# BUTSpeechFIT/TS-ASR-Whisper

Hardware: AMD Instinct MI355X
Metric: train utterances/sec (30 s clips) whisper-large-v3-turbo DiCoW (higher is better)
Workload: dtype bf16; 1 GPU; whisper-large-v3-turbo DiCoW fine-tune step, per-GPU batch 16, L=128, decoder frozen, bf16 AMP; global_batch=16, parallelism=dp1, split_streams=False, trainable_params=637306880

## Files before the change

### include/dicow_hip.h

```cpp
#ifndef DICOW_HIP_H
#define DICOW_HIP_H

#include <stdint.h>

#ifdef __cplusplus
extern "C" {
#endif

#define DICOW_OK 0
#define DICOW_ERR_INVALID (-1)
#define DICOW_ERR_LAUNCH (-2)

#define DICOW_ABI_VERSION 7

int dicow_abi_version(void);
int dicow_set_gemm_cus(int n);
int dicow_gemm_dispatch_log(char* buf, int cap);
const char* dicow_last_error(void);

int dicow_cast_f32_to_bf16(const float* src, void* dst, int64_t n, void* stream);
int dicow_cast_transpose_f32_to_bf16(const float* src, void* dst, int64_t ld, void* dst_t, int64_t ld_t, int R, int C,
                                     void* stream);
#define DICOW_CAST_GROUP_MAX 8
typedef struct { const float* src; void* dst; void* dst_t; int R, C; int64_t ld, ld_t; } dicow_cast_problem;
// ... 205 lines not shown
int dicow_fabric_emulate(void* buf, int64_t bytes, double gbps, int workgroups, int passes, void* stream);
int dicow_adamw_f32(float* p, const float* g, float* m, float* v, int64_t n, float lr, float beta1, float beta2,
                    float eps, float weight_decay, int step, const float* gnorm_sq, float max_norm, void* stream);
int dicow_adamw_hyper(int* counters, float* hyper, const int* is_pre, int n_runs, int preheat_only, double lr, double mult,
                      int warmup_steps, int max_steps, int cosine, double beta1, double beta2, void* stream);
int dicow_adamw_f32_dev(float* p, const float* g, float* m, float* v, int64_t n, const float* hyper, float beta1, float beta2,
                        float eps, float weight_decay, const float* gnorm_sq, float max_norm, void* stream);

#define DICOW_MT_CHUNK 2048
#define DICOW_MT_MAX_CLASSES 32
#define DICOW_MT_ALIGNED_ALL 1
#define DICOW_MT_ALIGNED_G   2
typedef struct {
    float* p; float* g; float* m; float* v;
    int64_t n;
    int32_t cls;
    int32_t flags;
} dicow_mt_tensor;
typedef struct { int64_t start; int32_t tensor; int32_t len; } dicow_mt_chunk;
typedef struct {
    float decay[DICOW_MT_MAX_CLASSES]; float step_size[DICOW_MT_MAX_CLASSES]; float bc2_sqrt[DICOW_MT_MAX_CLASSES];
    float lerp_w[DICOW_MT_MAX_CLASSES]; float beta2[DICOW_MT_MAX_CLASSES]; float one_minus_beta2[DICOW_MT_MAX_CLASSES];
    float eps[DICOW_MT_MAX_CLASSES];
    int32_t n_classes;
} dicow_mt_adamw_classes;
int dicow_multi_chunk_elems(void);
int dicow_multi_adamw_f32(const dicow_mt_tensor* tensors, const dicow_mt_chunk* chunks, int64_t n_chunks,
                          const dicow_mt_adamw_classes* cls, int cls_base, const float* clip_coef, void* stream);
int64_t dicow_multi_sumsq_ws_bytes(int64_t n_chunks);
int dicow_multi_sumsq_f32(const dicow_mt_tensor* tensors, const dicow_mt_chunk* chunks, int64_t n_chunks, void* ws, int64_t ws_bytes,
                          float* out, float max_norm, void* stream);
int dicow_multi_scale_f32(const dicow_mt_tensor* tensors, const dicow_mt_chunk* chunks, int64_t n_chunks, const float* coef, void* stream);


#ifdef DICOW_EXPERIMENTAL_ABI
#define DICOW_EPI_LNSTAT  2048
#define DICOW_EPI_LNFOLD  4096
#define DICOW_LN_SLOTS 16
int dicow_gemm_nt_lnstat_ok(const dicow_gemm_args* a);
int dicow_lnfold_prep(const float* W, const float* gamma, const float* beta, const float* bias, void* Wf, int64_t ldw, float* c, float* bf,
                      int N, int K, void* stream);
#endif

#ifdef __cplusplus
}
#endif
#endif
```

### ts-asr-whisper_amd/_lib.py

```python
import ctypes as C
import os

_HERE = os.path.dirname(os.path.abspath(__file__))
LIB_PATH = os.environ.get("DICOW_HIP_LIB") or os.path.join(_HERE, "libdicow_hip.so")
_lib = None

c_vp, c_i, c_i64, c_f, c_d = C.c_void_p, C.c_int, C.c_int64, C.c_float, C.c_double


class FddtLnFwdArgs(C.Structure):
    _fields_ = [("h_in", c_vp), ("in_bf16", c_i), ("mode", c_i), ("stno", c_vp), ("stno_bstride", c_i64),
                ("w", c_vp * 4), ("b", c_vp * 4), ("pos", c_vp), ("h_out", c_vp), ("ln_w", c_vp), ("ln_b", c_vp),
                ("y_bf16", c_vp), ("y_f32", c_vp), ("mean", c_vp), ("rstd", c_vp),
                ("rows", c_i), ("T", c_i), ("D", c_i), ("eps", c_f)]


class FddtLnBwdArgs(C.Structure):
    _fields_ = [("h_in", c_vp), ("in_bf16", c_i), ("mode", c_i), ("stno", c_vp), ("stno_bstride", c_i64),
                ("w", c_vp * 4), ("b", c_vp * 4), ("pos", c_vp), ("ln_w", c_vp), ("mean", c_vp), ("rstd", c_vp),
                ("d_y", c_vp), ("dy_f32", c_i), ("g_res", c_vp), ("g_out", c_vp), ("g_out_bf16", c_vp),
                ("dln_w", c_vp), ("dln_b", c_vp), ("dw", c_vp * 4), ("db", c_vp * 4), ("colsum_out", c_vp),
                ("dpos_rows", c_vp), ("rows", c_i), ("T", c_i), ("D", c_i), ("ws", c_vp), ("ws_bytes", c_i64)]


# ... 98 lines not shown
    "dicow_fddt_full_combine_bwd": [c_vp, c_vp, c_i64, c_i, c_vp, c_vp, c_i, c_i, c_i, c_vp],
    "dicow_gemm_nt": [C.POINTER(GemmArgs), c_vp],
    "dicow_gemm_nt_is_persistent": [C.POINTER(GemmArgs)],
    "dicow_gemm_tn": [C.POINTER(GemmTnArgs), c_vp],
    "dicow_gemm_tn_group": [C.POINTER(GemmTnGroupArgs), c_vp],
    "dicow_attn_fwd": [C.POINTER(AttnFwdArgs), c_vp],
    "dicow_attn_bwd": [C.POINTER(AttnBwdArgs), c_vp],
    "dicow_attn_bwd_fused_status": [c_vp],
    "dicow_ce_loss_fwd": [C.POINTER(CeArgs), c_vp],
    "dicow_ce_loss_bwd": [C.POINTER(CeArgs), c_vp, c_vp],
    "dicow_ctc_loss_fwd": [C.POINTER(CtcArgs), c_vp],
    "dicow_ctc_loss_bwd": [C.POINTER(CtcArgs), c_vp, c_vp],
    "dicow_embed_fwd": [c_vp, c_vp, c_vp, c_vp, c_i, c_i, c_i, c_vp],
    "dicow_embed_bwd": [c_vp, c_vp, c_vp, c_vp, c_i, c_i, c_i, c_vp],
    "dicow_gelu_bwd_bf16": [c_vp, c_vp, c_vp, c_i64, c_vp],
    "dicow_conv2_col2im_gelu_bwd": [c_vp, c_vp, c_vp, c_i, c_i, c_i, c_vp],
    "dicow_logmel": [c_vp, c_i, c_i, c_vp, c_vp, c_vp, c_vp, c_i, c_vp, c_vp, c_i64, c_vp],
    "dicow_stno_noise_rescale": [c_vp, c_vp, c_vp, c_i, c_i, c_i, c_f, c_vp],
    "dicow_stno_segment_augment": [c_vp, c_vp, c_vp, c_i, c_i, c_i, c_vp],
    "dicow_specaug_joint": [c_vp, c_vp, c_vp, c_vp, c_i, c_i, c_i, c_i, c_i, c_i, c_vp, c_i, c_vp, c_i, c_i, c_vp],
    "dicow_ctc_frame_lse": [c_vp, c_i, c_i64, c_i, c_i64, c_vp, c_vp],
    "dicow_ctc_prefix_init": [c_vp, c_i, c_i64, c_vp, c_i, c_i, c_i, c_vp, c_vp],
    "dicow_ctc_prefix_score": [C.POINTER(CtcPrefixArgs), c_vp],
    "dicow_whisper_timestamp_rules": [c_vp, c_i64, c_i, c_i, c_vp, c_i, c_i, c_i, c_i, c_i, c_i, c_i, c_vp],
    "dicow_sumsq_f32": [c_vp, c_i64, c_vp, c_vp],
    "dicow_fabric_emulate": [c_vp, c_i64, c_d, c_i, c_i, c_vp],
    "dicow_adamw_f32": [c_vp, c_vp, c_vp, c_vp, c_i64, c_f, c_f, c_f, c_f, c_f, c_i, c_vp, c_f, c_vp],
    "dicow_adamw_hyper": [c_vp, c_vp, c_vp, c_i, c_i, c_d, c_d, c_i, c_i, c_i, c_d, c_d, c_vp],
    "dicow_adamw_f32_dev": [c_vp, c_vp, c_vp, c_vp, c_i64, c_vp, c_f, c_f, c_f, c_f, c_vp, c_f, c_vp],
    "dicow_multi_chunk_elems": [],
    "dicow_multi_adamw_f32": [c_vp, c_vp, c_i64, C.POINTER(MtAdamwClasses), c_i, c_vp, c_vp],
    "dicow_multi_sumsq_f32": [c_vp, c_vp, c_i64, c_vp, c_i64, c_vp, c_f, c_vp],
    "dicow_multi_scale_f32": [c_vp, c_vp, c_i64, c_vp, c_vp],
}


_SIGS_EXPERIMENTAL = {
    "dicow_gemm_nt_lnstat_ok": [C.POINTER(GemmArgs)],
    "dicow_lnfold_prep": [c_vp, c_vp, c_vp, c_vp, c_vp, c_i64, c_vp, c_vp, c_i, c_i, c_vp],
}


class DicowError(RuntimeError):
    pass


def lib():
    global _lib
    if _lib is None:
        if not os.path.exists(LIB_PATH):
            raise DicowError(f"{LIB_PATH} is missing: build it with ts-asr-whisper_amd/csrc/build.sh "
                             "(or __graft_entry__.build()); there is no CPU fallback")
        l = C.CDLL(LIB_PATH)
        l.dicow_abi_version.restype = c_i
        l.dicow_last_error.restype = C.c_char_p
        for name, at in _SIGS.items():
            fn = getattr(l, name)
            fn.argtypes = at
            fn.restype = c_i
        for name, at in _SIGS64.items():
            fn = getattr(l, name)
            fn.argtypes = at
            fn.restype = c_i64
        for name, at in _SIGS_STR.items():
            fn = getattr(l, name)
            fn.argtypes = at
# ... 65 lines not shown
```

### ts-asr-whisper_amd/csrc/elementwise.hip

```cpp
#include <stdarg.h>
#include "common.h"

static thread_local char g_err[512] = "";

void dicow_set_error(const char* fmt, ...) {
    va_list ap;
    va_start(ap, fmt);
    vsnprintf(g_err, sizeof(g_err), fmt, ap);
    va_end(ap);
}

extern "C" int dicow_abi_version(void) { return DICOW_ABI_VERSION; }
extern "C" const char* dicow_last_error(void) { return g_err; }

__global__ void cast_f32_bf16_kernel(const float* __restrict__ src, unsigned short* __restrict__ dst, int64_t n) {
    const int64_t n4 = n >> 2;
    const int64_t stride = (int64_t)gridDim.x * blockDim.x;
    for (int64_t i = (int64_t)blockIdx.x * blockDim.x + threadIdx.x; i < n4; i += stride) {
        const float4 v = reinterpret_cast<const float4*>(src)[i];
        reinterpret_cast<uint2*>(dst)[i] = make_uint2(pack_bf16x2(v.x, v.y), pack_bf16x2(v.z, v.w));
    }
    for (int64_t i = (n4 << 2) + (int64_t)blockIdx.x * blockDim.x + threadIdx.x; i < n; i += stride)
        dst[i] = f2bfbits(src[i]);
}

extern "C" int dicow_cast_f32_to_bf16(const float* src, void* dst, int64_t n, void* stream) {
    DICOW_REQUIRE(src && dst && n > 0, "cast_f32_to_bf16: bad args");
    int grid = (int)((n / 4 + 255) / 256);
    if (grid < 1) grid = 1;
    if (grid > 4096) grid = 4096;
    hipLaunchKernelGGL(cast_f32_bf16_kernel, dim3(grid), dim3(256), 0, (hipStream_t)stream, src, (unsigned short*)dst, n);
    DICOW_CHECK_LAUNCH("cast_f32_to_bf16");
    return DICOW_OK;
// ... 216 lines not shown
        }
        reinterpret_cast<float4*>(out)[i] = s;
    }
}
struct reduce_multi_args { float* out[11]; };
__global__ void reduce_parts_tall_kernel(const float* __restrict__ part, int nparts, int64_t stride, int64_t kstride,
                                         reduce_multi_args outs, int64_t n) {
    __shared__ float red[16][17];
    float* out = outs.out[blockIdx.y];
    if (!out) return;
    part += (int64_t)blockIdx.y * kstride;
    const int c = threadIdx.x & 15, pl = threadIdx.x >> 4;
    const int64_t j = (int64_t)blockIdx.x * 16 + c;
    float s = 0.f;
    if (j < n) {
        int p = pl;
        for (; p + 48 < nparts; p += 64) {
            const float a0 = part[(int64_t)p * stride + j], a1 = part[(int64_t)(p + 16) * stride + j];
            const float a2 = part[(int64_t)(p + 32) * stride + j], a3 = part[(int64_t)(p + 48) * stride + j];
            s += (a0 + a1) + (a2 + a3);
        }
        for (; p < nparts; p += 16) s += part[(int64_t)p * stride + j];
    }
    red[pl][c] = s;
    __syncthreads();
    if (pl == 0 && j < n) {
        float t = 0.f;
#pragma unroll
        for (int q = 0; q < 16; ++q) t += red[q][c];
        out[j] += t;
    }
}

int dicow_launch_reduce_multi(const float* part, int nparts, int64_t stride, int64_t kstride, float* const* outs, int nout,
                              int64_t n, hipStream_t st) {
#ifdef DICOW_SKIP_REDUCE_MULTI
    return DICOW_OK;
#endif
    reduce_multi_args ra;
    for (int k = 0; k < 11; ++k) ra.out[k] = k < nout ? outs[k] : nullptr;
    hipLaunchKernelGGL(reduce_parts_tall_kernel, dim3((unsigned)((n + 15) / 16), nout), dim3(256), 0, st, part, nparts, stride,
                       kstride, ra, n);
    DICOW_CHECK_LAUNCH("reduce_parts_multi");
    return DICOW_OK;
}

int dicow_launch_reduce_parts(const float* part, int nparts, int64_t stride, float* out, int64_t n, hipStream_t st) {
    if (nparts <= 16 && n % 4 == 0 && stride % 4 == 0) {
        int grid = (int)((n / 4 + 255) / 256); if (grid > 4096) grid = 4096; if (grid < 1) grid = 1;
        hipLaunchKernelGGL(reduce_parts_wide_kernel, dim3(grid), dim3(256), 0, st, part, nparts, stride, out, n / 4);
    } else {
        float* outs[1] = {out};
        return dicow_launch_reduce_multi(part, nparts, stride, 0, outs, 1, n, st);
    }
    DICOW_CHECK_LAUNCH("reduce_parts");
    return DICOW_OK;
}

__global__ void colsum_bf16_kernel(const unsigned short* __restrict__ x, int64_t ld, float* __restrict__ part, int rows, int N) {
    const int c = (blockIdx.x * blockDim.x + threadIdx.x) * 2;
    if (c >= N) return;
    float s0 = 0.f, s1 = 0.f;
    const int r1 = (int)(((int64_t)rows * (blockIdx.y + 1)) / gridDim.y);
    for (int r = (int)(((int64_t)rows * blockIdx.y) / gridDim.y); r < r1; ++r) {
        const unsigned u = *reinterpret_cast<const unsigned*>(x + (int64_t)r * ld + c);
        s0 += __uint_as_float(u << 16);
        s1 += __uint_as_float(u & 0xffff0000u);
    }
    *reinterpret_cast<float2*>(part + (int64_t)blockIdx.y * N + c) = make_float2(s0, s1);
}

static int colsum_slices(int rows, int N) {
    const int gx = dicow_cdiv(N, 512);
    int gy = 2048 / gx; if (gy < 1) gy = 1; if (gy > rows) gy = rows; if (gy > 512) gy = 512;
    return gy;
}

extern "C" int64_t dicow_colsum_ws_bytes(int rows, int N) { return (int64_t)colsum_slices(rows, N) * N * 4; }

extern "C" int dicow_colsum_bf16(const void* x, int64_t ld, float* out, int rows, int N, void* ws, int64_t ws_bytes, void* stream) {
    DICOW_REQUIRE(x && out && rows > 0 && N > 0 && N % 2 == 0 && ld % 2 == 0, "colsum_bf16: bad args (N, ld must be even)");
    const int gx = dicow_cdiv(N, 512), gy = colsum_slices(rows, N);
    DICOW_REQUIRE(ws && ws_bytes >= (int64_t)gy * N * 4, "colsum_bf16: workspace too small (need %ld bytes)", (long)gy * N * 4);
    hipLaunchKernelGGL(colsum_bf16_kernel, dim3(gx, gy), dim3(256), 0, (hipStream_t)stream, (const unsigned short*)x, ld, (float*)ws, rows, N);
    DICOW_CHECK_LAUNCH("colsum_bf16");
    return dicow_launch_reduce_parts((const float*)ws, gy, N, out, N, (hipStream_t)stream);
}

__global__ void sum_over_batch_kernel(const float* __restrict__ g, float* __restrict__ out, int B, int64_t TD) {
// ... 463 lines not shown
```

### ts-asr-whisper_amd/engine.py

```python
import contextlib
import os
from types import SimpleNamespace as NS

import torch

from . import _lib as L
from . import ops

BF16, F32 = torch.bfloat16, torch.float32
CLS = ("silence_linear", "target_linear", "non_target_linear", "overlap_linear")


def _e(shape, dtype, dev):
    return torch.empty(shape, dtype=dtype, device=dev)


def _ceil(a, b):
    return (a + b - 1) // b * b


WGRAD_SIDE_STREAM = os.environ.get("DICOW_WGRAD_STREAM", "0") == "1"
WGRAD_STREAM_PRIORITY = int(os.environ.get("DICOW_WGRAD_STREAM_PRIORITY", "-1"))
_WGRAD_STREAMS = {}


def wgrad_stream(dev):
    cur = torch.cuda.current_stream(dev)
    key = (dev.index, cur.cuda_stream)
    st = _WGRAD_STREAMS.get(key)
    if st is None:
        st = _WGRAD_STREAMS[key] = torch.cuda.Stream(device=dev, priority=WGRAD_STREAM_PRIORITY)
    return st


SPLIT_FWD = os.environ.get("DICOW_SPLIT_FWD", "1") != "0"
SPLIT_FWD_MIN_ROWS = int(os.environ.get("DICOW_SPLIT_FWD_MIN_ROWS", "16000"))
SPLIT_DEC = os.environ.get("DICOW_SPLIT_DEC", "1") != "0"
SPLIT_BWD = os.environ.get("DICOW_SPLIT_BWD", "1") != "0"
SPLIT_BWD_WGRAD = os.environ.get("DICOW_SPLIT_BWD_WGRAD", "alt")
SPLIT_BWD_MEM_FRACTION = float(os.environ.get("DICOW_SPLIT_BWD_MEM_FRACTION", "0.6"))
SPLIT_IN_CAPTURE = os.environ.get("DICOW_SPLIT_IN_CAPTURE", "0") == "1"
SPLIT_FWD_PARTS = int(os.environ.get("DICOW_SPLIT_FWD_PARTS", "2"))
_FWD_STREAMS = {}


def _split_allowed():
    return SPLIT_IN_CAPTURE or not torch.cuda.is_current_stream_capturing()


def fwd_side_stream(dev, k=0):
    cur = torch.cuda.current_stream(dev)
    key = (dev.index, cur.cuda_stream, k)
    st = _FWD_STREAMS.get(key)
    if st is None:
        st = _FWD_STREAMS[key] = torch.cuda.Stream(device=dev, priority=-1)
    return st


def _fwd_parts(B, T, dev):
    n = SPLIT_FWD_PARTS if (SPLIT_FWD_PARTS > 2 and B % SPLIT_FWD_PARTS == 0) else 2
    main_st, Bp = torch.cuda.current_stream(dev), B // n
    parts = []
    for k in range(n):
        st = main_st if k == 0 else fwd_side_stream(dev, k - 1)
        if k:
            st.wait_stream(main_st)
        parts.append((st, slice(k * Bp * T, (k + 1) * Bp * T), slice(k * Bp, (k + 1) * Bp)))
    return main_st, parts, Bp


class GradSink:

    def __init__(self, params, dev, extra_rows=None):
        self.index, self.direct = {}, {}
        off = 0
        extra_rows = extra_rows or {}
# ... 618 lines not shown
        ops.scb_gate_bwd(g, s.upd, gate_p.detach(), d_upd, G.get(gate_p), Bp, T, D)
        tng = ops.TnGroup()
        bias_grad(d_upd, G.get(blk.ffn[3].bias))
        linear_wgrad(d_upd, s.a, G.get(blk.ffn[3].weight), rp, group=tng)
        d_u = linear_dgrad(d_upd, w.f3, rp, aux=s.u)
        bias_grad(d_u, G.get(blk.ffn[0].bias))
        linear_wgrad(d_u, s.cat, G.get(blk.ffn[0].weight), rp, group=tng)
        d_cat = linear_dgrad(d_u, w.f0, rp)
        d_attn = d_cat[:, :D]
        att = blk.cross_attn
        bias_grad(d_attn, G.get(att.out_proj.bias))
        linear_wgrad(d_attn, s.o, G.get(att.out_proj.weight), rp, group=tng)
        d_o = _e((rp, D), BF16, dev)
        ops.gemm_nt(d_attn, w.att.o.wt, d_o, rp, D, D, lda=2 * D)
        dq = _e((rp, D), BF16, dev)
        dkv = _e((rp, 2 * D), BF16, dev)
        delta = _e((2, Bp, H, T), F32, dev)
        ops.attn_bwd(heads(s.q, Bp, T, H), heads(s.kv[:, :D], Bp, T, H), heads(s.kv[:, D:], Bp, T, H), heads(s.o, Bp, T, H),
                     heads(d_o, Bp, T, H), s.lse, delta, heads(dq, Bp, T, H), heads(dkv[:, :D], Bp, T, H),
                     heads(dkv[:, D:], Bp, T, H), dq_scale=0.125, q_log2=QK_LOG2)
        bias_grad(dq, G.get(att.q_proj.bias))
        bias_grad(dkv[:, D:], G.get(att.v_proj.bias))
        linear_wgrad(dq, s.q_in, G.get(att.q_proj.weight), rp, group=tng)
        linear_wgrad(dkv[:, :D], s.kv_in, G.get(att.k_proj.weight), rp, group=tng)
        linear_wgrad(dkv[:, D:], s.kv_in, G.get(att.v_proj.weight), rp, group=tng)
        tng.run()
        d_qin = linear_dgrad(dq, w.att.q, rp, out_dtype=F32)
        d_kvin = linear_dgrad(dkv, w.att.kv, rp, out_dtype=F32)
        gin = _e((2 * rp, D), F32, dev)
        ops.scb_merge_bwd(g, d_qin, d_cat, d_kvin, gin, Bp, T, D)
        return gin

    def backward(self, S, d_enc, G):
        enc, cfg, W = self.enc, self.cfg, self.W
        dev = d_enc.device
        T, D, H, F_ = S.T, cfg.d_model, cfg.encoder_attention_heads, cfg.encoder_ffn_dim
        rows = S.B_out * T
        nl = len(enc.layers)
        g = _e((rows, D), F32, dev)
        gb = _e((rows, D), BF16, dev)
        last = enc.layers[nl - 1]
        sync = getattr(enc, "_split_sync", None)
        enter = sync.enter if sync is not None else (lambda name: None)
        enter("final_ln")
        ops.fddt_ln_bwd(S.h_last, rows, D, mode=ops.MODE_NONE, ln_w=enc.layer_norm.weight.detach(), mean=S.meanf, rstd=S.rstdf,
                        d_y=d_enc.contiguous(), g_out=g, g_out_bf16=gb, dln_w=G.get(enc.layer_norm.weight),
                        dln_b=G.get(enc.layer_norm.bias), colsum_out=G.get(last.fc2.bias))
        seg_hook = getattr(enc, "_segment_hook", None) or (lambda name: None)

        def hook(name):
            seg_hook(name)
            if sync is not None:
                sync.done(name)
        hook("final_ln")
        start = nl - 1
        if (SPLIT_BWD and SPLIT_FWD and getattr(S, "split_from", None) is not None and (sync is None or sync.role is None) and not WGRAD_SIDE_STREAM
                and S.B_out % 2 == 0 and _split_allowed() and self._split_bwd_fits(S, d_enc.device)):
            g, gb = self._backward_split(S, g, gb, G, hook)
            start = S.split_from - 1
            if start < 0:
                enter("stem")
                self._stem_backward(S, g, G)
                hook("stem")
                return
        tng, pend, ncu, per_layer = ops.TnGroup(), [], ops.num_cus(dev), 0
        side = wgrad_stream(dev) if (WGRAD_SIDE_STREAM and d_enc.is_cuda and not torch.cuda.is_current_stream_capturing()) else None

        def run_wgrads(names):
            if side is None or not tng.items:
                tng.run()
                for name in names:
                    hook(name)
                return
            ready = torch.cuda.Event()
            ready.record()
            held = [t for it in tng.items for t in (it[0], it[1], it[2])] + ([G.flat] if G.flat.numel() > 1 else [])
            with torch.cuda.stream(side):
                side.wait_event(ready)
                for t in held:
                    if t is not None and t.is_cuda:
                        t.record_stream(side)
                tng.run()
                for name in names:
                    hook(name)
        for i in range(start, -1, -1):
            n_before = len(tng.items)
            enter(f"layer{i}")
            lyr, w, Ls = enc.layers[i], W.layers[i], S.layers[i]
            rows, Bc = Ls.rows, Ls.B_after
            linear_wgrad(gb, Ls.a, G.get(lyr.fc2.weight), rows, group=tng, param=lyr.fc2.weight)
            d_u = linear_dgrad(gb, w.fc2, rows, aux=Ls.u, colsum_out=G.get(lyr.fc1.bias))
            linear_wgrad(d_u, Ls.xln2, G.get(lyr.fc1.weight), rows, group=tng, param=lyr.fc1.weight)
            d_xln2 = linear_dgrad(d_u, w.fc1, rows)
            g2 = _e((rows, D), F32, dev)
            g2b = _e((rows, D), BF16, dev)
            ln2 = lyr.final_layer_norm
            ops.fddt_ln_bwd(Ls.h2, rows, D, mode=ops.MODE_NONE, ln_w=ln2.weight.detach(), mean=Ls.mean2, rstd=Ls.rstd2,
                            d_y=d_xln2, g_res=g, g_out=g2, g_out_bf16=g2b, dln_w=G.get(ln2.weight), dln_b=G.get(ln2.bias),
                            colsum_out=G.get(lyr.self_attn.out_proj.bias))
            att = lyr.self_attn
            linear_wgrad(g2b, Ls.o, G.get(att.out_proj.weight), rows, group=tng, param=att.out_proj.weight)
            d_o = linear_dgrad(g2b, w.att.o, rows)
            d_qkv = _e((rows, 3 * D), BF16, dev)
            delta = _e((2, Bc, H, T), F32, dev)
            qkv = Ls.qkv
            ops.attn_bwd(heads(qkv[:, :D], Bc, T, H), heads(qkv[:, D:2 * D], Bc, T, H), heads(qkv[:, 2 * D:], Bc, T, H),
                         heads(Ls.o, Bc, T, H), heads(d_o, Bc, T, H), Ls.lse, delta, heads(d_qkv[:, :D], Bc, T, H),
                         heads(d_qkv[:, D:2 * D], Bc, T, H), heads(d_qkv[:, 2 * D:], Bc, T, H), dq_scale=0.125, q_log2=QK_LOG2,
                         dq_colsum=G.get(att.q_proj.bias), dv_colsum=G.get(att.v_proj.bias))
            qkv_wgrad(d_qkv, Ls.xln, G.get(att.q_proj.weight), G.get(att.k_proj.weight), G.get(att.v_proj.weight), rows, D, group=tng,
                      params=(att.q_proj.weight, att.k_proj.weight, att.v_proj.weight))
            d_xln = linear_dgrad(d_qkv, w.att.qkv, rows)
            fd = enc.fddts[i] if (cfg.use_fddt and i < len(enc.fddts)) else None
            mode, fw, fb = fddt_ptrs(fd, cfg)
            dw = tuple(G.get(x) for x in fw)
            db = tuple(G.get(x) for x in fb)
            ln = lyr.self_attn_layer_norm
            prev_b2 = G.get(enc.layers[i - 1].fc2.bias) if i > 0 else None
            rows_in = Ls.B * T
            g0 = _e((rows_in, D), F32, dev)
            g0b = _e((rows_in, D), BF16, dev) if i > 0 else None
            wfull = W.full[i] if (fd is not None and i < len(W.full)) else None
            if wfull is not None:
                gf = _e((rows, D), F32, dev)
                ops.fddt_ln_bwd(Ls.hp, rows, D, mode=ops.MODE_NONE, ln_w=ln.weight.detach(), mean=Ls.mean, rstd=Ls.rstd,
                                d_y=d_xln, g_res=g2, g_out=gf, dln_w=G.get(ln.weight), dln_b=G.get(ln.bias))
                if hasattr(Ls, "scb"):
                    if getattr(Ls, "dropped", False):
                        full = torch.zeros(rows_in, D, dtype=F32, device=dev)
                        full.view(Ls.B // 2, 2, T, D)[:, 0].copy_(gf.view(Ls.B // 2, T, D))
                        gf = full
                    gf = self._scb_bwd(i, Ls.scb, gf, G, T)
                g0 = full_fddt_bwd(fd, wfull, Ls.full_hb, gf, S.stno, Ls.bstride, G, rows_in, T, D)
                if i > 0:
                    g0b = ops.cast_bf16(g0)
                    if prev_b2 is not None:
                        ops.colsum_bf16(g0b, prev_b2)
            elif not hasattr(Ls, "scb"):
                ops.fddt_ln_bwd(Ls.h_in, rows, D, mode=mode, stno=S.stno, stno_bstride=Ls.bstride, T=T, w=fw, b=fb,
                                ln_w=ln.weight.detach(), mean=Ls.mean, rstd=Ls.rstd, d_y=d_xln, g_res=g2, g_out=g0,
                                g_out_bf16=g0b, dln_w=G.get(ln.weight), dln_b=G.get(ln.bias), dw=dw, db=db,
                                colsum_out=prev_b2)
            else:
                gs = _e((rows, D), F32, dev)
                ops.fddt_ln_bwd(Ls.hp, rows, D, mode=ops.MODE_NONE, ln_w=ln.weight.detach(), mean=Ls.mean, rstd=Ls.rstd,
                                d_y=d_xln, g_res=g2, g_out=gs, dln_w=G.get(ln.weight), dln_b=G.get(ln.bias))
                if getattr(Ls, "dropped", False):
                    full = torch.zeros(rows_in, D, dtype=F32, device=dev)
                    full.view(Ls.B // 2, 2, T, D)[:, 0].copy_(gs.view(Ls.B // 2, T, D))
                    gs = full
                gin = self._scb_bwd(i, Ls.scb, gs, G, T)
                ops.fddt_ln_bwd(Ls.h_in, rows_in, D, mode=mode, stno=S.stno, stno_bstride=Ls.bstride, T=T, w=fw, b=fb,
                                g_res=gin, g_out=g0, g_out_bf16=g0b, dw=dw, db=db, colsum_out=prev_b2)
            g, gb = g0, g0b
            pend.append(f"layer{i}")
            per_layer = max(per_layer, len(tng.items) - n_before)
            if i == 0 or tng.tiles() >= ncu or len(tng.items) + per_layer > L.TN_GROUP_MAX:
                run_wgrads(pend)
                pend = []
        enter("stem")
        self._stem_backward(S, g, G)
        if side is not None:
            torch.cuda.current_stream(dev).wait_stream(side)
        hook("stem")

    def _split_bwd_fits(self, S, dev):
        cfg = self.cfg
        nl = len(self.enc.layers) - S.split_from
        need = nl * S.B_out * S.T * (2 * cfg.encoder_ffn_dim + 24 * cfg.d_model + 64)
        if not dev.type == "cuda":
            return True
        total = getattr(self, "_dev_total_mem", None)
        if total is None:
            total = self._dev_total_mem = torch.cuda.get_device_properties(dev).total_memory
        free = total - torch.cuda.memory_allocated(dev)
        return need < SPLIT_BWD_MEM_FRACTION * free

    def _shadow(self, G, dev):
        enc, cfg = self.enc, self.cfg
        sh = getattr(self, "_sh", None)
        if sh is None or sh.flat.device != dev:
            per, off = [], 0
            for i, lyr in enumerate(enc.layers):
                ps = [p for p in lyr.parameters() if p.dim() == 1]
                fd = enc.fddts[i] if (cfg.use_fddt and i < len(enc.fddts)) else None
                if fd is not None:
                    ps += [p for p in fd.parameters() if p.dim() == 1]
                per.append(ps)
                off += sum(_ceil(p.numel(), 64) for p in ps)
            sh = NS(flat=torch.zeros(max(off, 1), dtype=F32, device=dev), view={}, per=per)
            off = 0
            for ps in per:
                for p in ps:
                    sh.view[id(p)] = sh.flat[off:off + p.numel()].view(p.shape)
                    off += _ceil(p.numel(), 64)
            self._sh = sh
        sh.flat.zero_()

        def get(p):
            if p is None or G.get(p) is None:
                return None
            return sh.view[id(p)]
        return sh, get

    def _backward_split(self, S, g, gb, G, hook):
        enc, cfg, W = self.enc, self.cfg, self.W
        dev = g.device
        T, D, H, F_ = S.T, cfg.d_model, cfg.encoder_attention_heads, cfg.encoder_ffn_dim
        nl = len(enc.layers)
        Bc = S.B_out
        rows = Bc * T
        main_st, parts, Bh = _fwd_parts(Bc, T, dev)
        side_st = parts[1][0]
        rh = Bh * T
        sh, shget = self._shadow(G, dev)
        side_st.wait_stream(main_st)
        keep, pending = [], None

        third_st = wgrad_stream(dev) if SPLIT_BWD_WGRAD == "third" else None
        deferred = []

        def settle(item):
            i, ev_side, ev3 = item
            main_st.wait_event(ev_side)
            main_st.wait_event(ev3)
            dst = [G.get(p) for p in sh.per[i]]
            src = [sh.view[id(p)] for p, d in zip(sh.per[i], dst) if d is not None]
            dst = [d for d in dst if d is not None]
            if dst:
                torch._foreach_add_(dst, src)
            hook(f"layer{i}")

        def finish(item):
            i, tg, ev_main, ev_side = item
            if third_st is not None:
                with torch.cuda.stream(third_st):
                    third_st.wait_event(ev_main)
                    third_st.wait_event(ev_side)
                    tg.run()
                    ev3 = third_st.record_event()
                deferred.append((i, ev_side, ev3))
                if len(deferred) > 1:
                    settle(deferred.pop(0))
                return
            if SPLIT_BWD_WGRAD == "alt" and (i & 1):
                with torch.cuda.stream(side_st):
                    side_st.wait_event(ev_main)
                    tg.run()
                    ev_side = side_st.record_event()
                main_st.wait_event(ev_side)
            else:
                main_st.wait_event(ev_side)
                tg.run()
            dst = [G.get(p) for p in sh.per[i]]
            src = [sh.view[id(p)] for p, d in zip(sh.per[i], dst) if d is not None]
            dst = [d for d in dst if d is not None]
            if dst:
                torch._foreach_add_(dst, src)
            hook(f"layer{i}")

        lo, sstep = S.split_from, S.split_sstep
        for i in range(nl - 1, lo - 1, -1):
            lyr, w, Ls = enc.layers[i], W.layers[i], S.layers[i]
            att, ln, ln2 = lyr.self_attn, lyr.self_attn_layer_norm, lyr.final_layer_norm
            fd = enc.fddts[i] if (cfg.use_fddt and i < len(enc.fddts)) else None
            mode, fw, fb = fddt_ptrs(fd, cfg)
            prev_b2 = enc.layers[i - 1].fc2.bias if i > 0 else None
            d_u, d_xln2 = _e((rows, F_), BF16, dev), _e((rows, D), BF16, dev)
            g2, g2b, d_o = _e((rows, D), F32, dev), _e((rows, D), BF16, dev), _e((rows, D), BF16, dev)
            d_qkv, d_xln = _e((rows, 3 * D), BF16, dev), _e((rows, D), BF16, dev)
            g0, g0b = _e((rows, D), F32, dev), (_e((rows, D), BF16, dev) if i > 0 else None)
            keep += [d_u, d_xln2, g2, g2b, d_o, d_qkv, d_xln, g0, g0b, g, gb]
            qkv = Ls.qkv
            evs = []
            for k, (st_, r, bsl) in enumerate(parts):
                gg = G.get if k == 0 else shget
                with torch.cuda.stream(st_):
                    linear_dgrad(gb[r], w.fc2, rh, aux=Ls.u[r], colsum_out=gg(lyr.fc1.bias), out=d_u[r])
                    linear_dgrad(d_u[r], w.fc1, rh, out=d_xln2[r])
                    ops.fddt_ln_bwd(Ls.h2[r], rh, D, mode=ops.MODE_NONE, ln_w=ln2.weight.detach(), mean=Ls.mean2[r], rstd=Ls.rstd2[r],
                                    d_y=d_xln2[r], g_res=g[r], g_out=g2[r], g_out_bf16=g2b[r], dln_w=gg(ln2.weight), dln_b=gg(ln2.bias),
                                    colsum_out=gg(att.out_proj.bias))
                    linear_dgrad(g2b[r], w.att.o, rh, out=d_o[r])
                    delta = _e((2, Bh, H, T), F32, dev)
                    ops.attn_bwd(heads(qkv[r][:, :D], Bh, T, H), heads(qkv[r][:, D:2 * D], Bh, T, H), heads(qkv[r][:, 2 * D:], Bh, T, H),
                                 heads(Ls.o[r], Bh, T, H), heads(d_o[r], Bh, T, H), Ls.lse[bsl], delta, heads(d_qkv[r][:, :D], Bh, T, H),
                                 heads(d_qkv[r][:, D:2 * D], Bh, T, H), heads(d_qkv[r][:, 2 * D:], Bh, T, H), dq_scale=0.125, q_log2=QK_LOG2,
                                 dq_colsum=gg(att.q_proj.bias), dv_colsum=gg(att.v_proj.bias))
                    linear_dgrad(d_qkv[r], w.att.qkv, rh, out=d_xln[r])
                    ops.fddt_ln_bwd(Ls.h_in[r], rh, D, mode=mode, stno=S.stno[bsl.start * sstep:], stno_bstride=Ls.bstride, T=T, w=fw, b=fb,
                                    ln_w=ln.weight.detach(), mean=Ls.mean[r], rstd=Ls.rstd[r], d_y=d_xln[r], g_res=g2[r], g_out=g0[r],
                                    g_out_bf16=g0b[r] if g0b is not None else None, dln_w=gg(ln.weight), dln_b=gg(ln.bias),
                                    dw=tuple(gg(x) for x in fw), db=tuple(gg(x) for x in fb), colsum_out=gg(prev_b2))
                    keep.append(delta)
                    evs.append(st_.record_event())
            tg = ops.TnGroup()
            linear_wgrad(gb, Ls.a, G.get(lyr.fc2.weight), rows, group=tg, param=lyr.fc2.weight)
            linear_wgrad(d_u, Ls.xln2, G.get(lyr.fc1.weight), rows, group=tg, param=lyr.fc1.weight)
            linear_wgrad(g2b, Ls.o, G.get(att.out_proj.weight), rows, group=tg, param=att.out_proj.weight)
            qkv_wgrad(d_qkv, Ls.xln, G.get(att.q_proj.weight), G.get(att.k_proj.weight), G.get(att.v_proj.weight), rows, D, group=tg,
                      params=(att.q_proj.weight, att.k_proj.weight, att.v_proj.weight))
            if pending is not None:
                finish(pending)
            pending = (i, tg, evs[0], evs[1])
            g, gb = g0, g0b
        finish(pending)
        while deferred:
            settle(deferred.pop(0))
        main_st.wait_stream(side_st)
        if third_st is not None:
            main_st.wait_stream(third_st)
        if lo > 0:
            pb = enc.layers[lo - 1].fc2.bias
            if G.get(pb) is not None:
                G.get(pb).add_(sh.view[id(pb)])
        del keep
        return g, gb

    def _stem_backward(self, S, g, G):
        enc, cfg, W = self.enc, self.cfg, self.W
        dev = g.device
        T, D = S.T, cfg.d_model
        B, Tin, M = S.B0, 2 * T, cfg.num_mel_bins
        rows = B * T
        gpos = G.get(enc.embed_positions.weight)
        if gpos is not None:
            ops.sum_over_batch(g.view(B, T * D), gpos)
        conv_train = enc.conv1.weight.requires_grad or enc.conv2.weight.requires_grad or enc.conv1.bias.requires_grad
        init_fddt = enc.initial_fddt if (cfg.use_fddt and cfg.use_pre_pos_fddt) else None
        mode, fw, fb = fddt_ptrs(init_fddt, cfg)
        dw = tuple(G.get(x) for x in fw)
        db = tuple(G.get(x) for x in fb)
        if not conv_train and all(x is None for x in dw + db):
            return
        if W.full_init is not None:
            d_x2 = ops.cast_bf16(full_fddt_bwd(init_fddt, W.full_init, S.x2b, g, S.stno, 4 * T, G, rows, T, D))
        else:
            d_x2 = _e((rows, D), BF16, dev)
            ops.fddt_ln_bwd(S.x2, rows, D, mode=mode, stno=S.stno, T=T, w=fw, b=fb, g_res=g, g_out_bf16=d_x2, dw=dw, db=db)
        if not conv_train:
            return
        conv_stem_bwd(enc, W, S.stem, d_x2, G)


class DecoderEngine:
# ... 375 lines not shown
```

### ts-asr-whisper_amd/ops.py

```python
import ctypes as C
import os
from typing import Optional, Sequence

import torch

from . import _lib as L

BF16 = torch.bfloat16
F32 = torch.float32


def _req(t: torch.Tensor, dtype, name: str):
    if not t.is_cuda:
        raise L.DicowError(f"{name}: tensor must live on the GPU (no CPU fallback)")
    if t.dtype != dtype:
        raise L.DicowError(f"{name}: expected {dtype}, got {t.dtype}")
    return t


def _p(t):
    return None if t is None else t.data_ptr()


_WS = {}


def workspace(nbytes: int, device) -> torch.Tensor:
    key = (device.type, device.index, torch.cuda.current_stream(device).cuda_stream if device.type == "cuda" else 0)
    t = _WS.get(key)
    if t is None or t.numel() < nbytes:
        t = torch.empty(max(nbytes, 64 << 20), dtype=torch.uint8, device=device)
        _WS[key] = t
    return t


def gemm_dispatch_log() -> dict:
    n = L.lib().dicow_gemm_dispatch_log(None, 0)
    buf = C.create_string_buffer(n + 64)
    L.lib().dicow_gemm_dispatch_log(buf, n + 64)
    out = {}
    for line in buf.value.decode().splitlines():
        k, _, c = line.partition("\t")
        out[k] = int(c)
    return out


_NCU = {}


def num_cus(device=None) -> int:
    dev = torch.cuda.current_device() if device is None else torch.device(device).index
    if dev not in _NCU:
        _NCU[dev] = torch.cuda.get_device_properties(dev).multi_processor_count
    lim = L.lib().dicow_set_gemm_cus(0)
    L.lib().dicow_set_gemm_cus(lim)
    return lim if 0 < lim < _NCU[dev] else _NCU[dev]


def set_gemm_cus(n: int) -> int:
    return L.lib().dicow_set_gemm_cus(int(n))


def _arr4(ts):
    a = (C.c_void_p * 4)()
    for i, t in enumerate(ts):
        a[i] = None if t is None else t.data_ptr()
# ... 440 lines not shown
```

Measured before the change: 123.8 utt/s.

## Defer per-layer bias/LN vector reductions into one batched settle kernel

Adds a thread-local collector that records the partial-sum reductions produced during each encoder layer's backward (bias colsums, LN/FDDT vector grads) instead of launching them one by one. When the layer ends, a single settle kernel sums all recorded parts into their outputs. In the split-stream path this also replaces the shadow-gradient buffers and foreach_add with per-stream arena workspaces held in a ring. Partial buffers come from ring-allocated arenas so they stay live until the deferred kernel runs. The aim is fewer kernel launches and no extra shadow-accumulate pass, at the cost of added memory, cross-stream event bookkeeping and more complex state handling.

```diff
diff --git a/include/dicow_hip.h b/include/dicow_hip.h
--- a/include/dicow_hip.h
+++ b/include/dicow_hip.h
@@ -261,6 +261,14 @@
                           float* out, float max_norm, void* stream);
 int dicow_multi_scale_f32(const dicow_mt_tensor* tensors, const dicow_mt_chunk* chunks, int64_t n_chunks, const float* coef, void* stream);
 
+int dicow_settle_begin(void);
+int dicow_settle_end(void);
+int dicow_settle_abandon(void);
+int dicow_settle_run(void* stream);
+int dicow_settle_from_zero(int on);
+int dicow_settle_stat(int what);
+int dicow_reduce_parts(const float* part, int nparts, int64_t stride, int64_t kstride, float* const* outs, int nout, int64_t n, void* stream);
+
 
 #ifdef DICOW_EXPERIMENTAL_ABI
 #define DICOW_EPI_LNSTAT  2048
diff --git a/ts-asr-whisper_amd/_lib.py b/ts-asr-whisper_amd/_lib.py
--- a/ts-asr-whisper_amd/_lib.py
+++ b/ts-asr-whisper_amd/_lib.py
@@ -154,6 +154,13 @@
     "dicow_multi_adamw_f32": [c_vp, c_vp, c_i64, C.POINTER(MtAdamwClasses), c_i, c_vp, c_vp],
     "dicow_multi_sumsq_f32": [c_vp, c_vp, c_i64, c_vp, c_i64, c_vp, c_f, c_vp],
     "dicow_multi_scale_f32": [c_vp, c_vp, c_i64, c_vp, c_vp],
+    "dicow_settle_begin": [],
+    "dicow_settle_end": [],
+    "dicow_settle_abandon": [],
+    "dicow_settle_run": [c_vp],
+    "dicow_settle_from_zero": [c_i],
+    "dicow_settle_stat": [c_i],
+    "dicow_reduce_parts": [c_vp, c_i, c_i64, c_i64, c_vp, c_i, c_i64, c_vp],
 }
 
 
diff --git a/ts-asr-whisper_amd/csrc/elementwise.hip b/ts-asr-whisper_amd/csrc/elementwise.hip
--- a/ts-asr-whisper_amd/csrc/elementwise.hip
+++ b/ts-asr-whisper_amd/csrc/elementwise.hip
@@ -1,4 +1,7 @@
 #include <stdarg.h>
+#include <atomic>
+#include <deque>
+#include <vector>
 #include "common.h"
 
 static thread_local char g_err[512] = "";
@@ -281,11 +284,152 @@
     }
 }
 
+enum { SETTLE_TALL = 0, SETTLE_WIDE = 1, SETTLE_WIDE_ZERO = 2 };
+#define SETTLE_MAX_TASKS 48
+struct settle_task { const float* part; float* out; int64_t stride; int64_t n; int nparts; int mode; };
+struct settle_args {
+    settle_task t[SETTLE_MAX_TASKS];
+    int blk0[SETTLE_MAX_TASKS + 1];
+    int first[SETTLE_MAX_TASKS];
+    int ntasks, nouts;
+};
+static_assert(sizeof(settle_args) <= 2560, "settle_args travels in the kernel arguments: keep it small");
+
+__global__ void __launch_bounds__(256) settle_parts_kernel(const settle_args a) {
+    __shared__ float red[16][17];
+    int o = 0;
+    while (o + 1 < a.nouts && (int)blockIdx.x >= a.blk0[o + 1]) ++o;
+    const int c = threadIdx.x & 15, pl = threadIdx.x >> 4;
+    const int64_t j = (int64_t)((int)blockIdx.x - a.blk0[o]) * 16 + c;
+    float* const out = a.t[a.first[o]].out;
+    float acc = 0.f;
+    if (pl == 0 && j < a.t[a.first[o]].n) acc = out[j];
+    for (int k = a.first[o]; k < a.ntasks; ++k) {
+        if (a.t[k].out != out) continue;
+        const float* __restrict__ part = a.t[k].part;
+        const int nparts = a.t[k].nparts, mode = a.t[k].mode;
+        const int64_t stride = a.t[k].stride;
+        if (mode != SETTLE_TALL) {
+            if (pl == 0 && j < a.t[k].n) {
+                float s = mode == SETTLE_WIDE ? acc : 0.f;
+                for (int p = 0; p < nparts; ++p) s += part[(int64_t)p * stride + j];
+                acc = mode == SETTLE_WIDE ? s : acc + s;
+            }
+            continue;
+        }
+        float s = 0.f;
+        if (j < a.t[k].n) {
+            int p = pl;
+            for (; p + 48 < nparts; p += 64) {
+                const float a0 = part[(int64_t)p * stride + j], a1 = part[(int64_t)(p + 16) * stride + j];
+                const float a2 = part[(int64_t)(p + 32) * stride + j], a3 = part[(int64_t)(p + 48) * stride + j];
+                s += (a0 + a1) + (a2 + a3);
+            }
+            for (; p < nparts; p += 16) s += part[(int64_t)p * stride + j];
+        }
+        __syncthreads();
+        red[pl][c] = s;
+        __syncthreads();
+        if (pl == 0) {
+            float t = 0.f;
+#pragma unroll
+            for (int q = 0; q < 16; ++q) t += red[q][c];
+            acc += t;
+        }
+    }
+    if (pl == 0 && j < a.t[a.first[o]].n) out[j] = acc;
+}
+
+struct settle_state {
+    bool open = false, from_zero = false;
+    std::vector<settle_task> cur;
+    std::vector<int> cur_records;
+    std::deque<std::vector<settle_task>> sealed;
+    std::deque<int> sealed_records;
+};
+static thread_local settle_state g_settle;
+static std::atomic<int> g_settle_launches{0};
+
+static int settle_launch(const settle_task* t, int nt, hipStream_t st) {
+    settle_args a;
+    a.ntasks = nt; a.nouts = 0;
+    int blocks = 0;
+    for (int k = 0; k < nt; ++k) {
+        a.t[k] = t[k];
+        bool seen = false;
+        for (int o = 0; o < a.nouts && !seen; ++o) seen = a.t[a.first[o]].out == t[k].out;
+        if (seen) continue;
+        a.first[a.nouts] = k; a.blk0[a.nouts] = blocks; ++a.nouts;
+        blocks += (int)((t[k].n + 15) / 16);
+    }
+    a.blk0[a.nouts] = blocks;
+    hipLaunchKernelGGL(settle_parts_kernel, dim3(blocks), dim3(256), 0, st, a);
+    DICOW_CHECK_LAUNCH("settle_parts");
+    ++g_settle_launches;
+    return DICOW_OK;
+}
+
+static int settle_record(const float* part, int nparts, int64_t stride, int64_t kstride, float* const* outs, int nout, int64_t n, int mode) {
+    settle_state& S = g_settle;
+    DICOW_REQUIRE(part && nparts > 0 && n > 0 && nout >= 0 && nout <= 11, "settle: bad record");
+    for (int k = 0; k < nout; ++k)
+        for (const settle_task& t : S.cur) DICOW_REQUIRE(t.out != outs[k] || t.n == n, "settle: one output recorded with two lengths");
+    for (int k = 0; k < nout; ++k)
+        if (outs[k]) S.cur.push_back({part + (int64_t)k * kstride, outs[k], stride, n, nparts, mode});
+    S.cur_records.push_back((int)S.cur.size());
+    return DICOW_OK;
+}
+
+extern "C" int dicow_settle_begin(void) {
+    DICOW_REQUIRE(!g_settle.open, "settle_begin: a collector is already open on this thread");
+    g_settle.open = true; g_settle.from_zero = false;
+    return DICOW_OK;
+}
+extern "C" int dicow_settle_end(void) {
+    settle_state& S = g_settle;
+    DICOW_REQUIRE(S.open, "settle_end: no collector is open on this thread");
+    S.open = false; S.from_zero = false;
+    S.sealed.push_back(std::move(S.cur)); S.sealed_records.push_back((int)S.cur_records.size());
+    S.cur.clear(); S.cur_records.clear();
+    return DICOW_OK;
+}
+extern "C" int dicow_settle_abandon(void) {
+    settle_state& S = g_settle;
+    S.open = false; S.from_zero = false;
+    S.cur.clear(); S.cur_records.clear(); S.sealed.clear(); S.sealed_records.clear();
+    return DICOW_OK;
+}
+extern "C" int dicow_settle_from_zero(int on) {
+    DICOW_REQUIRE(g_settle.open, "settle_from_zero: no collector is open on this thread");
+    g_settle.from_zero = on != 0;
+    return DICOW_OK;
+}
+extern "C" int dicow_settle_run(void* stream) {
+    settle_state& S = g_settle;
+    if (S.sealed.empty()) return DICOW_OK;
+    const std::vector<settle_task> t = std::move(S.sealed.front());
+    S.sealed.pop_front(); S.sealed_records.pop_front();
+    for (size_t k = 0; k < t.size(); k += SETTLE_MAX_TASKS) {
+        const size_t nt = t.size() - k < SETTLE_MAX_TASKS ? t.size() - k : SETTLE_MAX_TASKS;
+        if (const int rc = settle_launch(t.data() + k, (int)nt, (hipStream_t)stream)) return rc;
+    }
+    return DICOW_OK;
+}
+extern "C" int dicow_settle_stat(int what) {
+    const settle_state& S = g_settle;
+    int n = (int)S.cur_records.size();
+    switch (what) {
+        case 0: for (int r : S.sealed_records) n += r; return n;
+        case 1: return S.open ? 1 : 0;
+        case 2: return (int)S.sealed.size();
+        case 3: return g_settle_launches.load();
+        default: return -1;
+    }
+}
+
 int dicow_launch_reduce_multi(const float* part, int nparts, int64_t stride, int64_t kstride, float* const* outs, int nout,
                               int64_t n, hipStream_t st) {
-#ifdef DICOW_SKIP_REDUCE_MULTI
-    return DICOW_OK;
-#endif
+    if (g_settle.open) return settle_record(part, nparts, stride, kstride, outs, nout, n, SETTLE_TALL);
     reduce_multi_args ra;
     for (int k = 0; k < 11; ++k) ra.out[k] = k < nout ? outs[k] : nullptr;
     hipLaunchKernelGGL(reduce_parts_tall_kernel, dim3((unsigned)((n + 15) / 16), nout), dim3(256), 0, st, part, nparts, stride,
@@ -296,6 +440,10 @@
 
 int dicow_launch_reduce_parts(const float* part, int nparts, int64_t stride, float* out, int64_t n, hipStream_t st) {
     if (nparts <= 16 && n % 4 == 0 && stride % 4 == 0) {
+        if (g_settle.open) {
+            float* outs[1] = {out};
+            return settle_record(part, nparts, stride, 0, outs, 1, n, g_settle.from_zero ? SETTLE_WIDE_ZERO : SETTLE_WIDE);
+        }
         int grid = (int)((n / 4 + 255) / 256); if (grid > 4096) grid = 4096; if (grid < 1) grid = 1;
         hipLaunchKernelGGL(reduce_parts_wide_kernel, dim3(grid), dim3(256), 0, st, part, nparts, stride, out, n / 4);
     } else {
@@ -304,6 +452,16 @@
     }
     DICOW_CHECK_LAUNCH("reduce_parts");
     return DICOW_OK;
+}
+
+extern "C" int dicow_reduce_parts(const float* part, int nparts, int64_t stride, int64_t kstride, float* const* outs, int nout, int64_t n,
+                                  void* stream) {
+    DICOW_REQUIRE(part && outs && nparts > 0 && n > 0 && nout >= 1 && nout <= 11 && stride >= n, "reduce_parts: bad args");
+    if (nout == 1 && kstride == 0) {
+        DICOW_REQUIRE(outs[0], "reduce_parts: null output");
+        return dicow_launch_reduce_parts(part, nparts, stride, outs[0], n, (hipStream_t)stream);
+    }
+    return dicow_launch_reduce_multi(part, nparts, stride, kstride, outs, nout, n, (hipStream_t)stream);
 }
 
 __global__ void colsum_bf16_kernel(const unsigned short* __restrict__ x, int64_t ld, float* __restrict__ part, int rows, int N) {
diff --git a/ts-asr-whisper_amd/engine.py b/ts-asr-whisper_amd/engine.py
--- a/ts-asr-whisper_amd/engine.py
+++ b/ts-asr-whisper_amd/engine.py
@@ -42,6 +42,7 @@
 SPLIT_IN_CAPTURE = os.environ.get("DICOW_SPLIT_IN_CAPTURE", "0") == "1"
 SPLIT_FWD_PARTS = int(os.environ.get("DICOW_SPLIT_FWD_PARTS", "2"))
 _FWD_STREAMS = {}
+SETTLE_VECTORS = True
 
 
 def _split_allowed():
@@ -726,6 +727,19 @@
         return gin
 
     def backward(self, S, d_enc, G):
+        try:
+            self._backward_impl(S, d_enc, G)
+        except BaseException:
+            ops.settle_abandon()
+            raise
+
+    def _settle_bytes(self, rows, B, T):
+        cfg, lib = self.cfg, L.lib()
+        D, H, F_ = cfg.d_model, cfg.encoder_attention_heads, cfg.encoder_ffn_dim
+        return ops.settle_ws_bytes(lib.dicow_gemm_nt_colsum_ws_bytes(rows, F_), lib.dicow_fddt_ln_bwd_ws_bytes(rows, D),
+                                   lib.dicow_fddt_ln_bwd_ws_bytes(rows, D), lib.dicow_attn_bwd_colsum_ws_bytes(B, H, T, T))
+
+    def _backward_impl(self, S, d_enc, G):
         enc, cfg, W = self.enc, self.cfg, self.W
         dev = d_enc.device
         T, D, H, F_ = S.T, cfg.d_model, cfg.encoder_attention_heads, cfg.encoder_ffn_dim
@@ -782,6 +796,10 @@
             enter(f"layer{i}")
             lyr, w, Ls = enc.layers[i], W.layers[i], S.layers[i]
             rows, Bc = Ls.rows, Ls.B_after
+            defer = (SETTLE_VECTORS and not hasattr(Ls, "scb")
+                     and not (cfg.use_fddt and i < len(enc.fddts) and i < len(W.full) and W.full[i] is not None))
+            if defer:
+                ops.settle_begin(dev, self._settle_bytes(rows, Bc, T))
             linear_wgrad(gb, Ls.a, G.get(lyr.fc2.weight), rows, group=tng, param=lyr.fc2.weight)
             d_u = linear_dgrad(gb, w.fc2, rows, aux=Ls.u, colsum_out=G.get(lyr.fc1.bias))
             linear_wgrad(d_u, Ls.xln2, G.get(lyr.fc1.weight), rows, group=tng, param=lyr.fc1.weight)
@@ -846,6 +864,9 @@
                 gin = self._scb_bwd(i, Ls.scb, gs, G, T)
                 ops.fddt_ln_bwd(Ls.h_in, rows_in, D, mode=mode, stno=S.stno, stno_bstride=Ls.bstride, T=T, w=fw, b=fb,
                                 g_res=gin, g_out=g0, g_out_bf16=g0b, dw=dw, db=db, colsum_out=prev_b2)
+            if defer:
+                ops.settle_end()
+                ops.settle_run()
             g, gb = g0, g0b
             pend.append(f"layer{i}")
             per_layer = max(per_layer, len(tng.items) - n_before)
@@ -862,6 +883,8 @@
         cfg = self.cfg
         nl = len(self.enc.layers) - S.split_from
         need = nl * S.B_out * S.T * (2 * cfg.encoder_ffn_dim + 24 * cfg.d_model + 64)
+        if SETTLE_VECTORS and dev.type == "cuda":
+            need += ops.SETTLE_RING * 2 * self._settle_bytes(S.B_out // 2 * S.T, S.B_out // 2, S.T)
         if not dev.type == "cuda":
             return True
         total = getattr(self, "_dev_total_mem", None)
@@ -907,22 +930,31 @@
         main_st, parts, Bh = _fwd_parts(Bc, T, dev)
         side_st = parts[1][0]
         rh = Bh * T
-        sh, shget = self._shadow(G, dev)
-        side_st.wait_stream(main_st)
+        settle_v = SETTLE_VECTORS
+        arena_bytes = 2 * self._settle_bytes(rh, Bh, T) if settle_v else 0
+        if not settle_v:
+            sh, shget = self._shadow(G, dev)
+            side_st.wait_stream(main_st)
         keep, pending = [], None
 
         third_st = wgrad_stream(dev) if SPLIT_BWD_WGRAD == "third" else None
         deferred = []
 
-        def settle(item):
-            i, ev_side, ev3 = item
-            main_st.wait_event(ev_side)
-            main_st.wait_event(ev3)
+        def add_vectors(i):
+            if settle_v:
+                ops.settle_run()
+                return
             dst = [G.get(p) for p in sh.per[i]]
             src = [sh.view[id(p)] for p, d in zip(sh.per[i], dst) if d is not None]
             dst = [d for d in dst if d is not None]
             if dst:
                 torch._foreach_add_(dst, src)
+
+        def settle(item):
+            i, ev_side, ev3 = item
+            main_st.wait_event(ev_side)
+            main_st.wait_event(ev3)
+            add_vectors(i)
             hook(f"layer{i}")
 
         def finish(item):
@@ -946,11 +978,7 @@
             else:
                 main_st.wait_event(ev_side)
                 tg.run()
-            dst = [G.get(p) for p in sh.per[i]]
-            src = [sh.view[id(p)] for p, d in zip(sh.per[i], dst) if d is not None]
-            dst = [d for d in dst if d is not None]
-            if dst:
-                torch._foreach_add_(dst, src)
+            add_vectors(i)
             hook(f"layer{i}")
 
         lo, sstep = S.split_from, S.split_sstep
@@ -967,8 +995,12 @@
             keep += [d_u, d_xln2, g2, g2b, d_o, d_qkv, d_xln, g0, g0b, g, gb]
             qkv = Ls.qkv
             evs = []
+            if settle_v:
+                ops.settle_begin(dev, arena_bytes, side_streams=(side_st,))
             for k, (st_, r, bsl) in enumerate(parts):
-                gg = G.get if k == 0 else shget
+                gg = G.get if (k == 0 or settle_v) else shget
+                if settle_v:
+                    ops.settle_from_zero(k > 0)
                 with torch.cuda.stream(st_):
                     linear_dgrad(gb[r], w.fc2, rh, aux=Ls.u[r], colsum_out=gg(lyr.fc1.bias), out=d_u[r])
                     linear_dgrad(d_u[r], w.fc1, rh, out=d_xln2[r])
@@ -988,6 +1020,8 @@
                                     dw=tuple(gg(x) for x in fw), db=tuple(gg(x) for x in fb), colsum_out=gg(prev_b2))
                     keep.append(delta)
                     evs.append(st_.record_event())
+            if settle_v:
+                ops.settle_end()
             tg = ops.TnGroup()
             linear_wgrad(gb, Ls.a, G.get(lyr.fc2.weight), rows, group=tg, param=lyr.fc2.weight)
             linear_wgrad(d_u, Ls.xln2, G.get(lyr.fc1.weight), rows, group=tg, param=lyr.fc1.weight)
@@ -1004,7 +1038,7 @@
         main_st.wait_stream(side_st)
         if third_st is not None:
             main_st.wait_stream(third_st)
-        if lo > 0:
+        if lo > 0 and not settle_v:
             pb = enc.layers[lo - 1].fc2.bias
             if G.get(pb) is not None:
                 G.get(pb).add_(sh.view[id(pb)])
diff --git a/ts-asr-whisper_amd/ops.py b/ts-asr-whisper_amd/ops.py
--- a/ts-asr-whisper_amd/ops.py
+++ b/ts-asr-whisper_amd/ops.py
@@ -1,5 +1,6 @@
 import ctypes as C
 import os
+import threading
 from typing import Optional, Sequence
 
 import torch
@@ -26,12 +27,86 @@
 
 
 def workspace(nbytes: int, device) -> torch.Tensor:
+    arena = getattr(_SETTLE, "arena", None)
+    if arena is not None and arena.buf.device == device:
+        off = arena.off
+        if off + nbytes > arena.buf.numel():
+            raise L.DicowError(f"settle arena too small: {off} + {nbytes} of {arena.buf.numel()} bytes (settle_begin's nbytes)")
+        arena.off = off + (nbytes + 255) // 256 * 256
+        return arena.buf[off:off + nbytes]
     key = (device.type, device.index, torch.cuda.current_stream(device).cuda_stream if device.type == "cuda" else 0)
     t = _WS.get(key)
     if t is None or t.numel() < nbytes:
         t = torch.empty(max(nbytes, 64 << 20), dtype=torch.uint8, device=device)
         _WS[key] = t
     return t
+
+
+SETTLE_RING = 3
+_SETTLE = threading.local()
+_SETTLE_RINGS = {}
+
+
+class _Arena:
+    __slots__ = ("buf", "off", "event", "sides")
+
+
+def settle_ws_bytes(*sizes) -> int:
+    return sum((int(n) + 255) // 256 * 256 for n in sizes)
+
+
+def settle_begin(device, nbytes: int, side_streams=()):
+    key = (device.index, torch.cuda.current_stream(device).cuda_stream)
+    ring = _SETTLE_RINGS.get(key)
+    if ring is None:
+        ring = _SETTLE_RINGS[key] = [[None] * SETTLE_RING, 0]
+    k = ring[1]
+    ring[1] = (k + 1) % SETTLE_RING
+    arena = ring[0][k]
+    if arena is None or arena.buf.numel() < nbytes:
+        arena = ring[0][k] = _Arena()
+        arena.buf, arena.event = torch.empty(max(int(nbytes), 256), dtype=torch.uint8, device=device), None
+    if arena.event is not None:
+        for st in side_streams:
+            st.wait_event(arena.event)
+    arena.off, arena.sides = 0, bool(side_streams)
+    L.call("dicow_settle_begin")
+    _SETTLE.arena = arena
+
+
+def settle_from_zero(on: bool):
+    L.call("dicow_settle_from_zero", int(on))
+
+
+def settle_end():
+    arena, _SETTLE.arena = _SETTLE.arena, None
+    L.call("dicow_settle_end")
+    if getattr(_SETTLE, "queue", None) is None:
+        _SETTLE.queue = []
+    _SETTLE.queue.append(arena)
+
+
+def settle_run():
+    L.call("dicow_settle_run", L.stream())
+    q = getattr(_SETTLE, "queue", None)
+    if q:
+        arena = q.pop(0)
+        arena.event = torch.cuda.current_stream(arena.buf.device).record_event() if arena.sides else None
+
+
+def settle_abandon():
+    _SETTLE.arena, _SETTLE.queue = None, []
+    L.lib().dicow_settle_abandon()
+
+
+def settle_stat(what: int) -> int:
+    return L.lib().dicow_settle_stat(int(what))
+
+
+def reduce_parts(part: torch.Tensor, outs, n: int, nparts: int, stride: int, kstride: int = 0):
+    _req(part, F32, "reduce_parts.part")
+    arr = (C.c_void_p * len(outs))(*[_p(o) for o in outs])
+    L.call("dicow_reduce_parts", part.data_ptr(), nparts, stride, kstride, arr, len(outs), n, L.stream())
 
 
 def gemm_dispatch_log() -> dict:
```

Result: no change. 124.1 utt/s (median of 2 runs) (+0.2%).
